# Shuijing725/CrowdNav_Prediction_AttnGraph

Measured on NVIDIA H100. Metric: env_steps_per_s_ppo_rollout, higher is better.
Workload: dtype f32

## Files before the change

### crowdnav_prediction_attngraph_b200/csrc/cn_gemm_tc.cu

```cuda
#include "cn_gemm_tc.h"

__global__ void cn_split_f16_kernel(const float* __restrict__ src, float scale, __half* __restrict__ hi,
                                    __half* __restrict__ lo, size_t count) {
  const size_t i = (size_t)blockIdx.x * blockDim.x + threadIdx.x;
  if (i >= count) return;
  const float x = fminf(fmaxf(src[i] * scale, -65504.0f), 65504.0f);
  const __half h = __float2half_rn(x);
  hi[i] = h;
  lo[i] = __float2half_rn(x - __half2float(h));
}

namespace {

typedef CUresult (*EncodeFn)(CUtensorMap*, CUtensorMapDataType, cuuint32_t, void*, const cuuint64_t*, const cuuint64_t*,
                             const cuuint32_t*, const cuuint32_t*, CUtensorMapInterleave, CUtensorMapSwizzle,
                             CUtensorMapL2promotion, CUtensorMapFloatOOBfill);

EncodeFn get_encode() {
  static EncodeFn fn = nullptr;
  if (!fn) {
    void* sym = nullptr;
    cudaDriverEntryPointQueryResult qres;
    if (cudaGetDriverEntryPoint("cuTensorMapEncodeTiled", &sym, cudaEnableDefault, &qres) == cudaSuccess &&
        qres == cudaDriverEntryPointSuccess)
      fn = reinterpret_cast<EncodeFn>(sym);
  }
  return fn;
}

int halloc16(CnLaunchCtx* c, __half** ptr, size_t count) {
  float* q = nullptr;
  int rc = palloc(c, &q, (count + 1) / 2);
// ... 78 lines not shown
  if (!rc) rc = tc_store_maps(v, rows, K);
  return rc;
}

void split16(CnLaunchCtx* c, cudaStream_t st, const float* src, float scale, __half* hi, __half* lo, size_t count) {
  cn_split_f16_kernel<<<(unsigned)((count + 255) / 256), 256, 0, st>>>(src, scale, hi, lo, count);
  c->launches += 1;
}

int tc_set_attrs() {
  cudaError_t e = cudaSuccess;
  for (int act = CN_ACT_NONE; act <= CN_ACT_TANH; ++act)
    for (int out = TC_OUT_F32; out <= TC_OUT_BOTH; ++out) {
      if (e == cudaSuccess)
        e = cudaFuncSetAttribute(tc_kernel<256>(act, out), cudaFuncAttributeMaxDynamicSharedMemorySize, TcCfg<256>::kSmemBytes);
      if (e == cudaSuccess)
        e = cudaFuncSetAttribute(tc_kernel<64>(act, out), cudaFuncAttributeMaxDynamicSharedMemorySize, TcCfg<64>::kSmemBytes);
    }
  if (e == cudaSuccess)
    e = cudaFuncSetAttribute(cn_gemm_tc_kernel<64, true>, cudaFuncAttributeMaxDynamicSharedMemorySize, TcCfg<64>::kSmemBytes);
  if (e == cudaSuccess)
    e = cudaFuncSetAttribute(cn_gemm_tc_kernel<256, false, CN_ACT_NONE, TC_OUT_GRU>,
                             cudaFuncAttributeMaxDynamicSharedMemorySize, TcCfg<256>::kSmemBytes);
  if (e != cudaSuccess) return cn_set_error("cudaFuncSetAttribute(tc): %s", cudaGetErrorString(e));
  return 0;
}

void gemm_tc(CnLaunchCtx* c, cudaStream_t st, const TcMat& A, const TcMat& B, int M, int N, int K, int bn, const float* bias,
             int act, const TcOut& o, const int* m_ptr, int act_lo, int act_hi, const int* m0_ptr) {
  TcEpilogue ep;
  memset(&ep, 0, sizeof(ep));
  ep.bias = bias; ep.inv_scale = 1.0f / 64.0f; ep.act = act; ep.act_lo = act_lo; ep.act_hi = act_hi;
  ep.c32 = o.c32; ep.ldc = o.ldc; ep.out_hi = o.oh; ep.out_lo = o.ol; ep.ldh = o.ldh; ep.m_ptr = m_ptr; ep.m0_ptr = m0_ptr;
  {
    static const int nostore = (getenv("CN_DBG_NOSTORE") && getenv("CN_DBG_NOSTORE")[0] == '1') ? 1 : 0;
    ep.dbg_nostore = nostore;
  }
  if (A.box_k != tc_box_k(bn) || B.box_k != tc_box_k(bn)) {
    if (!c->launch_error) {
      c->launch_error = true;
      cn_set_error("gemm_tc in stage '%s': operand boxes %d / %d wide, the BN = %d instance loads %d",
                   c->cur_stage ? c->cur_stage : "?", A.box_k, B.box_k, bn, tc_box_k(bn));
    }
    return;
  }
  const int out_kind = (o.c32 ? TC_OUT_F32 : 0) | (o.oh ? TC_OUT_F16 : 0);
// ... 35 lines not shown

void gemm_tc_gru(CnLaunchCtx* c, cudaStream_t st, const TcMat& A, const TcMat& B, int M, const float* bias,
                 const float* h_in, const float* mask, float* h_out, int group, int pitch, int off, __half* oh, __half* ol,
                 int ldh) {
  const int N = 4 * 256, K = 64 + 256;
  if (A.box_k != tc_box_k(256) || B.box_k != tc_box_k(256) || !bias || !h_out || !mask || group <= 0) {
    if (!c->launch_error) {
      c->launch_error = true;
      cn_set_error("gemm_tc_gru in stage '%s': operand boxes %d / %d wide (need %d), or a missing bias / mask / output",
                   c->cur_stage ? c->cur_stage : "?", A.box_k, B.box_k, tc_box_k(256));
    }
    return;
  }
  TcEpilogue ep;
  memset(&ep, 0, sizeof(ep));
  ep.bias = bias; ep.inv_scale = 1.0f / 64.0f; ep.act_hi = 1 << 30;
  ep.c32 = h_out; ep.ldc = 256; ep.out_hi = oh; ep.out_lo = ol; ep.ldh = ldh;
  ep.gru_h = h_in; ep.gru_mask = mask; ep.gru_group = group; ep.gru_pitch = pitch; ep.gru_off = off;
  static const CUtensorMap no_map = {};
  const int tiles = (N / 256) * ((M + TC_BM - 1) / TC_BM);
  dim3 grid(tiles < c->num_sms ? tiles : c->num_sms);
  launch_k(c, cn_gemm_tc_kernel<256, false, CN_ACT_NONE, TC_OUT_GRU>, grid, dim3(TC_THREADS), TcCfg<256>::kSmemBytes, st,
           A.mh, A.ml, B.mh, B.ml, M, N, K, ep, no_map, no_map, no_map);
}

int gemm_tc_promote(int num_sms, cudaStream_t st, const __half* ahi, const __half* alo, int a_rows, int a_pitch,
                    const __half* bhi, const __half* blo, int b_rows, int b_pitch, int Kd, float* C, int ldc,
                    const float* bias, int act, const float* inv_a, const float* inv_b, int ksplit) {
  const int bn = 64;
  if (b_rows % bn) return cn_set_error("cn_update gemm: output columns %d not a multiple of 64", b_rows);
  const int Kp = (Kd + TC_BK - 1) / TC_BK * TC_BK;
  CUtensorMap mah, mal, mbh, mbl;
  int rc = make_map(&mah, ahi, a_rows, Kd, TC_BM, a_pitch);
  if (!rc) rc = make_map(&mal, alo, a_rows, Kd, TC_BM, a_pitch);
  if (!rc) rc = make_map(&mbh, bhi, b_rows, Kd, bn, b_pitch);
  if (!rc) rc = make_map(&mbl, blo, b_rows, Kd, bn, b_pitch);
  if (rc) return rc;
  TcEpilogue ep;
  memset(&ep, 0, sizeof(ep));
  ep.bias = bias; ep.inv_scale = 1.0f; ep.act = act; ep.act_lo = 0; ep.act_hi = 1 << 30;
  ep.c32 = C; ep.ldc = ldc; ep.inv_scale_a = inv_a; ep.inv_scale_b = inv_b; ep.ksplit = ksplit;
  const int tiles = (b_rows / bn) * ((a_rows + TC_BM - 1) / TC_BM) * (ksplit > 1 ? ksplit : 1);
  const int grid = tiles < num_sms ? tiles : num_sms;
  static const CUtensorMap no_map = {};
  cn_gemm_tc_kernel<64, true><<<grid, TC_THREADS, TcCfg<64>::kSmemBytes, st>>>(mah, mal, mbh, mbl, a_rows, b_rows, Kp, ep,
                                                                                no_map, no_map, no_map);
// ... 29 lines not shown
  TcStoreMap sc, sh, sl;
  if (bn == 256) {
    if (!rc && dC) rc = make_store_map(&sc, dC, 4, M, N, N);
    if (!rc && out_hi) rc = make_store_map(&sh, out_hi, 2, M, N, ldh);
    if (!rc && out_hi) rc = make_store_map(&sl, out_lo, 2, M, N, ldh);
    o.sc = &sc; o.sh = &sh; o.sl = &sl;
  }
  if (!rc) {
    split16(&ctx, 0, dA, 1.0f, Af.hi, Af.lo, (size_t)M * a_pitch);
    split16(&ctx, 0, dW, 64.0f, B.hi, B.lo, (size_t)N * K);
    gemm_tc(&ctx, 0, A, B, M, N, K, bn, dbias, act, o, m_ptr, act_lo, act_hi > 0 ? act_hi : 1 << 30, m0_ptr);
    cudaError_t err = cudaDeviceSynchronize();
    if (err != cudaSuccess) rc = cn_set_error("cn_internal_gemm_tc_ex: %s", cudaGetErrorString(err));
    else if (ctx.launch_error) rc = 1;
  }
  cn_launch_free(&ctx);
  return rc;
}
int cn_internal_gemm_tc(const float* dA, const float* dW, const float* dbias, float* dC, int M, int N, int K, int act,
                        int bn) {
  return cn_internal_gemm_tc_ex(dA, dW, dbias, dC, M, N, K, act, bn, nullptr, nullptr, 0, 0, nullptr, nullptr, 0, 0, 0);
}

#ifdef CN_GEMM_TRACE
int cn_internal_gemm_trace(unsigned long long* dtrace, int cap) {
  g_tc_trace = dtrace; g_tc_trace_cap = dtrace ? cap : 0;
  return 0;
}
#endif

}
```

### crowdnav_prediction_attngraph_b200/csrc/cn_gemm_tc.cuh

```cuda
#pragma once
#include <cuda.h>
#include <cuda_fp16.h>
#include <cuda_runtime.h>
#include <stdint.h>

#include "cn_launch.cuh"

#define TC_BM 128
#define TC_BK 64
#define TC_CONSUMER_WARPS 8
#define TC_THREADS (128 + 32 * TC_CONSUMER_WARPS)

template <int BN>
struct TcCfg {
  static constexpr int kBK = (BN >= 256) ? 32 : TC_BK;
  static constexpr int kSwizzle = 2 * kBK;
  static constexpr int kStages = 4;
  static constexpr int kATile = TC_BM * kBK * 2;
  static constexpr int kBTile = BN * kBK * 2;
  static constexpr int kStageBytes = 2 * kATile + 2 * kBTile;
  static constexpr int kStoreBoxes = (BN >= 256) ? 2 : 0;
  static constexpr int kBoxBytes = 64 * 128;
  static constexpr int kStagingBytes = 2 * kStoreBoxes * kBoxBytes;
  static constexpr int kSmemBytes = kStages * kStageBytes + kStagingBytes + 256  + 1024 ;
// ... 384 lines not shown
#pragma unroll
      for (int k = 0; k < 2; ++k) {
        const int a = 4 * g + 2 * h + k;
        const float r = tc_sigmoid(fmaf(acc[a], inv_scale, __ldg(ep.bias + n0 + c + k)));
        const float z = tc_sigmoid(fmaf(acc[a + 32], inv_scale, __ldg(ep.bias + n0 + 64 + c + k)));
        const float gin = fmaf(acc[a + 64], inv_scale, __ldg(ep.bias + n0 + 128 + c + k));
        const float ghn = fmaf(acc[a + 96], inv_scale, __ldg(ep.bias + n0 + 192 + c + k));
        const float n = tanhf(gin + r * ghn);
        o[k] = (1.0f - z) * n + z * hv[k];
      }
      if (ep.dbg_nostore) continue;
      *reinterpret_cast<float2*>(ep.c32 + orow * 256 + u) = make_float2(o[0], o[1]);
      if (ep.out_hi) {
        uint32_t lo;
        const uint32_t hi = tc::split_pair_hi(o[0], o[1], &lo);
        const size_t q = (size_t)row * ep.ldh + u;
        *reinterpret_cast<uint32_t*>(ep.out_hi + q) = hi;
        *reinterpret_cast<uint32_t*>(ep.out_lo + q) = lo;
      }
    }
  }
}

template <int BN, bool PROMOTE = false, int ACT = 0, int OUT = TC_OUT_F32>
__global__ void __launch_bounds__(TC_THREADS, 1)
cn_gemm_tc_kernel(const __grid_constant__ CUtensorMap map_ahi, const __grid_constant__ CUtensorMap map_alo,
                  const __grid_constant__ CUtensorMap map_bhi, const __grid_constant__ CUtensorMap map_blo,
                  int M, int N, int K, TcEpilogue ep, const __grid_constant__ CUtensorMap map_c,
                  const __grid_constant__ CUtensorMap map_oh, const __grid_constant__ CUtensorMap map_ol) {
  cn_pdl_trigger();
  constexpr int TC_STAGES = TcCfg<BN>::kStages;
  constexpr int BK = TcCfg<BN>::kBK;
  constexpr int SW = TcCfg<BN>::kSwizzle;
  constexpr int TC_A_TILE_BYTES = TcCfg<BN>::kATile;
  constexpr int TC_B_TILE_BYTES = TcCfg<BN>::kBTile;
  constexpr int TC_STAGE_BYTES = TcCfg<BN>::kStageBytes;
  constexpr bool kTmaStore = !PROMOTE && BN == 256 && OUT != TC_OUT_GRU;
  static_assert(OUT != TC_OUT_GRU || (BN == 256 && !PROMOTE), "the GRU epilogue reads four 64-column gate blocks");
  static_assert(!PROMOTE || BK == 64, "PROMOTE sums 64-wide k-blocks");
  static_assert(!kTmaStore || TcCfg<BN>::kStoreBoxes > 0, "BN = 256 stages its output");
  extern __shared__ uint8_t tc_smem_raw[];
  const uint32_t raw = tc::smem_u32(tc_smem_raw);
  const uint32_t base = (raw + 1023u) & ~1023u;
  const uint32_t staging = base + TC_STAGES * TC_STAGE_BYTES;
  const uint32_t bar_base = staging + TcCfg<BN>::kStagingBytes;
  const uint32_t bar_full = bar_base, bar_empty = bar_base + 64;

  const int warp = threadIdx.x >> 5, lane = threadIdx.x & 31, wg = warp >> 2;
  const int num_kb = K / BK;

  if (threadIdx.x == 0) {
    for (int s = 0; s < TC_STAGES; ++s) {
      tc::mbar_init(bar_full + 8 * s, 1);
      tc::mbar_init(bar_empty + 8 * s, TC_CONSUMER_WARPS);
    }
    asm volatile("fence.mbarrier_init.release.cluster;" ::: "memory");
// ... 57 lines not shown
  sg.box = 0; sg.leader = (threadIdx.x & 127) == 0; sg.bar_id = wg;
  TC_TRACE(sg.waits = 0; sg.wait_clk = 0;)
  TC_TRACE(const bool tr = ep.trace && warp == 4 && lane == 0; int tr_n = 0;)
  for (int tile = blockIdx.x; tile < n_tiles; tile += gridDim.x) {
    const int mn = tile % n_mn, ks = tile / n_mn;
    const int m0 = m_lo + (mn / n_ntiles) * TC_BM, n0 = (mn % n_ntiles) * BN;
    const int kb0 = ks * kb_per, kb1 = (kb0 + kb_per < num_kb) ? kb0 + kb_per : num_kb;
    TC_TRACE(const uint64_t t_tile = tc::globaltimer(); uint64_t t_first = 0; uint32_t polls = 0;)
    float acc[BN / 2];
    float sum[PROMOTE ? BN / 2 : 1];
    if constexpr (PROMOTE) {
#pragma unroll
      for (int i = 0; i < BN / 2; ++i) sum[i] = 0.0f;
    }
    uint32_t prev = 0;
    for (int kb = kb0; kb < kb1; ++kb, ++it) {
      const uint32_t s = it % TC_STAGES, ph = (it / TC_STAGES) & 1u;
#ifdef CN_GEMM_TRACE
      polls += tc::mbar_wait_polls(bar_full + 8 * s, ph);
      if (kb == kb0) t_first = tc::globaltimer();
#else
      tc::mbar_wait(bar_full + 8 * s, ph);
#endif
      const uint32_t st = base + s * TC_STAGE_BYTES;
      const uint32_t a_hi = st + half * (TC_A_TILE_BYTES / 2), a_lo = a_hi + TC_A_TILE_BYTES,
                     b_hi = st + 2 * TC_A_TILE_BYTES, b_lo = b_hi + TC_B_TILE_BYTES;
      tc::fence_regs(acc);
      tc::wgmma_fence();
#pragma unroll
      for (int k = 0; k < BK / 16; ++k) {
        const uint32_t koff = k * 32;
        const uint64_t dah = tc::make_desc<SW>(a_hi + koff), dal = tc::make_desc<SW>(a_lo + koff);
        const uint64_t dbh = tc::make_desc<SW>(b_hi + koff), dbl = tc::make_desc<SW>(b_lo + koff);
        const bool first = k == 0 && (PROMOTE || kb == kb0);
        tc::wgmma_f16<BN>(acc, dah, dbh, first ? 0u : 1u);
        tc::wgmma_f16<BN>(acc, dah, dbl, 1u);
        tc::wgmma_f16<BN>(acc, dal, dbh, 1u);
      }
      tc::wgmma_commit();
      tc::fence_regs(acc);
      if constexpr (PROMOTE) {
        tc::wgmma_wait<0>();
        tc::fence_regs(acc);
        __syncwarp();
        if (lane == 0) tc::mbar_arrive(bar_empty + 8 * s);
#pragma unroll
        for (int i = 0; i < BN / 2; ++i) sum[i] += acc[i];
      } else {
        tc::wgmma_wait<1>();
        if (kb != kb0) {
          __syncwarp();
          if (lane == 0) tc::mbar_arrive(bar_empty + 8 * prev);
        }
        prev = s;
      }
    }
    if constexpr (PROMOTE) {
#pragma unroll
      for (int i = 0; i < BN / 2; ++i) acc[i] = sum[i];
    } else {
      tc::wgmma_wait<0>();
      tc::fence_regs(acc);
      __syncwarp();
// ... 44 lines not shown
        if (ep.c32) {
          float* c = ep.c32 + (size_t)row * ep.ldc + col;
          if (ksplit > 1) {
            atomicAdd(c, v0);
            atomicAdd(c + 1, v1);
          } else {
            *reinterpret_cast<float2*>(c) = make_float2(v0, v1);
          }
        }
        if (ep.out_hi) {
          uint32_t lo;
          const uint32_t hi = tc::split_pair_hi(v0, v1, &lo);
          const size_t o = (size_t)row * ep.ldh + col;
          *reinterpret_cast<uint32_t*>(ep.out_hi + o) = hi;
          *reinterpret_cast<uint32_t*>(ep.out_lo + o) = lo;
        }
      }
    }
  }
  if constexpr (kTmaStore) {
    if (sg.leader) tc::bulk_wait_all();
  }
}
```

### crowdnav_prediction_attngraph_b200/csrc/cn_gemm_tc.h

```cpp
#pragma once
#include <cuda.h>
#include <cuda_fp16.h>
#include <cuda_runtime.h>
#include <stdint.h>

#include "cn_gemm_tc.cuh"
#include "cn_launch.cuh"

struct TcStoreMap {
  CUtensorMap map;
  int rows = 0, cols = 0;
};

struct TcMat {
  __half *hi = nullptr, *lo = nullptr;
  CUtensorMap mh, ml;
  int pitch = 0;
  int box_k = 0;
  TcStoreMap sh, sl;
};

struct TcOut {
  float* c32 = nullptr; int ldc = 0;
  __half *oh = nullptr, *ol = nullptr; int ldh = 0;
// ... 2 lines not shown
inline TcOut out32(float* c, int ldc, const TcStoreMap* sc = nullptr) { TcOut o; o.c32 = c; o.ldc = ldc; o.sc = sc; return o; }
inline TcOut out16(const TcMat& t) { TcOut o; o.oh = t.hi; o.ol = t.lo; o.ldh = t.pitch; o.sh = &t.sh; o.sl = &t.sl; return o; }
inline TcOut out_both(float* c, int ldc, const TcMat& t) { TcOut o = out16(t); o.c32 = c; o.ldc = ldc; return o; }

inline int tc_box_k(int bn) { return bn == 256 ? TcCfg<256>::kBK : TcCfg<64>::kBK; }

inline bool tma_store_ok(const void* ptr, size_t pitch_bytes) { return ((uintptr_t)ptr % 16) == 0 && pitch_bytes % 16 == 0; }

int make_map(CUtensorMap* map, const __half* ptr, int rows, int K, int box_rows, int pitch, int box_k = TC_BK);
int make_store_map(TcStoreMap* s, const void* ptr, int esize, int rows, int cols, int pitch);
int tc_alloc(CnLaunchCtx* c, TcMat& t, int rows, int K, int box_rows, int box_k);
int tc_view(TcMat& v, const TcMat& src, int col0, int rows, int K, int box_rows);
void split16(CnLaunchCtx* c, cudaStream_t st, const float* src, float scale, __half* hi, __half* lo, size_t count);
int tc_set_attrs();

void gemm_tc(CnLaunchCtx* c, cudaStream_t st, const TcMat& A, const TcMat& B, int M, int N, int K, int bn, const float* bias,
             int act, const TcOut& o, const int* m_ptr = nullptr, int act_lo = 0, int act_hi = 1 << 30,
             const int* m0_ptr = nullptr);

void gemm_tc_gru(CnLaunchCtx* c, cudaStream_t st, const TcMat& A, const TcMat& B, int M, const float* bias,
                 const float* h_in, const float* mask, float* h_out, int group, int pitch, int off, __half* oh, __half* ol,
                 int ldh);

int gemm_tc_promote(int num_sms, cudaStream_t st, const __half* ahi, const __half* alo, int a_rows, int a_pitch,
                    const __half* bhi, const __half* blo, int b_rows, int b_pitch, int Kd, float* C, int ldc,
                    const float* bias, int act, const float* inv_a, const float* inv_b, int ksplit);
```

### crowdnav_prediction_attngraph_b200/csrc/cn_policy.cu

```cuda
#include <cuda_runtime.h>
#include <stdio.h>
#include <stdlib.h>
#include <string.h>
#include <map>
#include <string>
#include <vector>

#include "../../include/crowdnav_b200.h"
#include "cn_host_util.h"
#include "cn_gemm_tc.h"
#include "cn_launch.cuh"
#include "cn_policy_kernels.cuh"
#include "cn_qkv_attn.cuh"

struct cn_policy {
  cn_policy_config cfg;
  int N, H, Win, M;
  CnLaunchCtx lc;
  bool fuse_qkv;
  TcMat tWqkvH;
  CUtensorMap qa_ah, qa_al, qa_bh, qa_bl;
  float* bqkvH = nullptr;
  int* tile_tab = nullptr;
  cudaEvent_t ev_tiles;
  void (*attn_kernel)(const float*, const int*, const int*, const int*, const int*, float*, __half*, __half*);
  int attn_warps;
  int qkv_chunks;
  bool finalized;
  std::map<std::string, std::vector<float>> host;
  size_t ws_allocs;
  float *W1, *b1, *W2, *b2, *Wqkv, *bqkv, *Wos, *bos;
  float *Wr, *br, *Wet, *bet, *WsT, *bs, *Wa, *ba, *Wih, *bih, *Whh, *bhh, *Wo, *bo;
  float *Woac, *boac;
  float *Wac1, *bac1, *Wa2, *ba2, *Wc2, *bc2, *wv_, *bv, *Wm, *bm, *logstd;
  TcMat tW2, tWqkv, tWos, tWet, tWsT, tWa, tWih, tWhh, tWo, tWac1, tWoac, tWa2, tWc2;
  TcMat tE1, tE2, tAo;
  TcMat tRs, tT1, tTe, tWv, tH0, tH1, tOut, tAc1, tA1, tC1;
  cudaStream_t st2, st3;
  cudaEvent_t ev_fork, ev_join, ev_fork2, ev_join2, ev_fork3, ev_join3;
  bool profile;
  std::vector<cudaEvent_t> ev;
  int *row_start, *row_env, *mc;
  float *x16, *e1, *e2, *qkv, *ao, *sout, *xr, *rs, *t1, *u, *wv, *h0, *gi, *gh, *outb, *ac1, *a2, *c2;
  TcStoreMap qkv_st, sout_st;
};

void cn_hr_attention_dense(CnLaunchCtx* c, cudaStream_t st, const float* s_out, const float* u, const float* te, int ldte,
                           int te_off, const float* b_s, int env_pitch, int env_off, int N, int H, float* wv,
                           __half* wv_hi, __half* wv_lo, int ldwh) {
  launch_k(c, cn_hr_attention_kernel<true>, dim3((N + 3) / 4), dim3(128), 0, st, s_out, u, te, ldte, te_off, b_s,
// ... 69 lines not shown
    return cn_set_error("cn_policy_create: unsupported dims N=%d H=%d input=%d", cfg->num_envs, cfg->human_num,
                        cfg->input_size);
  int ndev = 0;
  cudaError_t err = cudaGetDeviceCount(&ndev);
  if (err != cudaSuccess || ndev == 0)
    return cn_set_error("cn_policy_create: no CUDA device (%s); this engine has no CPU fallback",
                        err == cudaSuccess ? "device count 0" : cudaGetErrorString(err));
  if (cfg->device < 0 || cfg->device >= ndev) return cn_set_error("cn_policy_create: bad device %d", cfg->device);
  cudaSetDevice(cfg->device);
  cn_policy* p = new cn_policy();
  p->cfg = *cfg;
  p->N = cfg->num_envs; p->H = cfg->human_num; p->Win = cfg->input_size; p->M = p->N * p->H;
  p->finalized = false; p->profile = false;
  cn_launch_init(&p->lc, cfg->device);
  {
    const char* qc = getenv("CN_QKV_CHUNKS");
    p->qkv_chunks = (qc && qc[0] == '2') ? 2 : 1;
    const char* ar = getenv("CN_ATTN_R");
    const int attn_r = ar ? atoi(ar) : 1;
    p->attn_kernel = attn_r == 1 ? cn_hh_attention_kernel<1, 4, 4> : (attn_r == 4 ? cn_hh_attention_kernel<4, 2, 2> : cn_hh_attention_kernel<2, 4, 4>);
    p->attn_warps = attn_r == 4 ? 2 : 4;
    const char* fq = getenv("CN_FUSE_QKV");
    p->fuse_qkv = cfg->gemm_mode == 1 && p->qkv_chunks == 1 && (fq && fq[0] == '1') && p->N <= QA_MAX_ENVS && p->H <= 128;
  }
  cudaEventCreateWithFlags(&p->ev_tiles, cudaEventDisableTiming);
  cudaStreamCreateWithFlags(&p->st2, cudaStreamNonBlocking);
  cudaStreamCreateWithFlags(&p->st3, cudaStreamNonBlocking);
  cudaEventCreateWithFlags(&p->ev_fork3, cudaEventDisableTiming);
  cudaEventCreateWithFlags(&p->ev_join3, cudaEventDisableTiming);
  cudaEventCreateWithFlags(&p->ev_fork, cudaEventDisableTiming);
  cudaEventCreateWithFlags(&p->ev_join, cudaEventDisableTiming);
  cudaEventCreateWithFlags(&p->ev_fork2, cudaEventDisableTiming);
  cudaEventCreateWithFlags(&p->ev_join2, cudaEventDisableTiming);
  const size_t M = (size_t)p->M, N = (size_t)p->N;
  const int Mi = p->M, Ni = p->N;
  int rc = 0;
#define WS(name, count) if (!rc) rc = palloc(&p->lc, &p->name, (count))
  {
    float* q = nullptr;
    if (!rc) rc = palloc(&p->lc, &q, N + 2);
    p->row_start = reinterpret_cast<int*>(q);
    if (!rc) rc = palloc(&p->lc, &q, 4);
    p->mc = reinterpret_cast<int*>(q);
    if (!rc) rc = palloc(&p->lc, &q, M + 1);
    p->row_env = reinterpret_cast<int*>(q);
    if (!rc) rc = palloc(&p->lc, &q, 2 * N + 4);
    p->tile_tab = reinterpret_cast<int*>(q);
  }
  WS(x16, M * 16); WS(e1, M * 128); WS(e2, M * 512); WS(qkv, M * 1536); WS(ao, M * 512); WS(sout, M * 256);
  WS(xr, N * 16); WS(rs, N * 256); WS(t1, N * 128); WS(u, N * 256); WS(wv, N * 256); WS(h0, N * 128);
  WS(gi, N * 384); WS(gh, N * 384); WS(outb, N * 256); WS(ac1, N * 512); WS(a2, N * 256); WS(c2, N * 256);
#undef WS
  if (!rc && cfg->gemm_mode == 1) {
    rc = tc_alloc(&p->lc, p->tE1, Mi, 128, TC_BM, tc_box_k(256));
    if (!rc) rc = tc_alloc(&p->lc, p->tE2, Mi, 512, TC_BM, tc_box_k(256));
    if (!rc) rc = tc_alloc(&p->lc, p->tAo, Mi, 512, TC_BM, tc_box_k(256));
    if (!rc) rc = tc_alloc(&p->lc, p->tRs, Ni, 256, TC_BM, tc_box_k(64));
    if (!rc) rc = tc_alloc(&p->lc, p->tT1, Ni, 128, TC_BM, tc_box_k(64));
    if (!rc) rc = tc_view(p->tTe, p->tT1, 64, Ni, 64, TC_BM);
    if (!rc) rc = tc_alloc(&p->lc, p->tWv, Ni, 256, TC_BM, tc_box_k(64));
    if (!rc) rc = tc_alloc(&p->lc, p->tH0, Ni, 128, TC_BM, tc_box_k(64));
    if (!rc) rc = tc_alloc(&p->lc, p->tH1, Ni, 128, TC_BM, tc_box_k(64));
    if (!rc) rc = tc_alloc(&p->lc, p->tOut, Ni, 256, TC_BM, tc_box_k(64));
    if (!rc) rc = tc_alloc(&p->lc, p->tAc1, Ni, 512, TC_BM, tc_box_k(64));
    if (!rc) rc = tc_view(p->tA1, p->tAc1, 0, Ni, 256, TC_BM);
    if (!rc) rc = tc_view(p->tC1, p->tAc1, 256, Ni, 256, TC_BM);
    if (!rc) rc = make_store_map(&p->qkv_st, p->qkv, 4, Mi, 1536, 1536);
    if (!rc) rc = make_store_map(&p->sout_st, p->sout, 4, Mi, 256, 256);
    if (!rc) rc = tc_set_attrs();
    if (!rc) {
// ... 160 lines not shown
      split16(&p->lc, st, wh, 64.0f, p->tWqkvH.hi, p->tWqkvH.lo, (size_t)1536 * 512);
    }
  }
  cudaError_t err = cudaStreamSynchronize(st);
  if (err != cudaSuccess) return cn_set_error("cn_policy_finalize: %s", cudaGetErrorString(err));
  p->finalized = true;
  return 0;
}

int cn_policy_act(cn_policy* p, const cn_act_ptrs* d, void* stream) {
  if (!p || !d) return cn_set_error("cn_policy_act: null argument");
  if (!p->finalized) return cn_set_error("cn_policy_act: call cn_policy_finalize after setting parameters");
  if (!d->robot_node || !d->temporal_edges || !d->spatial_edges || !d->detected_human_num || !d->h_in || !d->masks ||
      !d->value || !d->action || !d->log_prob || !d->h_out)
    return cn_set_error("cn_policy_act: missing input/output pointer");
  CnDeviceGuard guard(p->cfg.device);
  cudaStream_t st = (cudaStream_t)stream;
  const int N = p->N, H = p->H, M = p->M;
  const bool tcm = p->cfg.gemm_mode == 1;
  const int* mc = p->mc;
  const int ALL = 1 << 30;
  mark(p, st, 0);
  {
    launch_k(&p->lc, cn_row_offsets_kernel, dim3(1), dim3(1024), 0, st, d->detected_human_num, N, H, p->row_start, p->mc);
    const int total = (!tcm && M * 16 > N * 128) ? M * 16 : N * 128;
    launch_k(&p->lc, cn_pack_inputs_kernel, dim3((total + 255) / 256), dim3(256), 0, st, d->spatial_edges, p->Win, H, N, p->row_start, p->row_env,
                                                               tcm ? nullptr : p->x16,
                                                               d->temporal_edges, d->robot_node, d->h_in, d->masks, p->xr,
                                                               p->h0, tcm ? p->tH0.hi : nullptr, tcm ? p->tH0.lo : nullptr);
  }
  cudaStream_t s2 = p->st2;
  cudaEventRecord(p->ev_fork, st);
  cudaStreamWaitEvent(s2, p->ev_fork, 0);
  if (p->fuse_qkv) {
    cn_qkv_tiles_kernel<<<1, 1024, 0, s2>>>(p->row_start, N, p->tile_tab);
    p->lc.launches += 1;
    cudaEventRecord(p->ev_tiles, s2);
  }
  if (tcm) {
    gemm(p, s2, p->xr, 16, p->Wr, 16, p->br, nullptr, 256, N, 256, 16, CN_ACT_RELU, 0, ALL, nullptr, p->tRs.hi, p->tRs.lo);
    gemm_tc(&p->lc, s2, p->tRs, p->tWet, N, 128, 256, 64, p->bet, CN_ACT_RELU, out_both(p->t1, 128, p->tT1), nullptr, 0, 64);
    gemm_tc(&p->lc, s2, p->tTe, p->tWsT, N, 256, 64, 64, nullptr, CN_ACT_NONE, out32(p->u, 256));
    gemm_tc(&p->lc, s2, p->tH0, p->tWhh, N, 384, 128, 64, p->bhh, CN_ACT_NONE, out32(p->gh, 384));
  } else {
    gemm(p, s2, p->xr, 16, p->Wr, 16, p->br, p->rs, 256, N, 256, 16, CN_ACT_RELU);
    gemm(p, s2, p->rs, 256, p->Wet, 256, p->bet, p->t1, 128, N, 128, 256, CN_ACT_RELU, 0, 64);
    gemm(p, s2, p->t1 + 64, 128, p->WsT, 64, nullptr, p->u, 256, N, 256, 64, CN_ACT_NONE);
    gemm(p, s2, p->h0, 128, p->Whh, 128, p->bhh, p->gh, 384, N, 384, 128, CN_ACT_NONE);
  }
  cudaEventRecord(p->ev_join, s2);
  mark(p, st, 1);
  if (tcm) {
    launch_k(&p->lc, cn_embed1_kernel, dim3(p->lc.num_sms * 6), dim3(256), 0, st, d->spatial_edges, p->Win, H, p->row_start, p->row_env, p->mc, p->W1, p->b1,
                                                     p->tE1.hi, p->tE1.lo);
  } else gemm(p, st, p->x16, 16, p->W1, 16, p->b1, p->e1, 128, M, 128, 16, CN_ACT_RELU, 0, ALL, mc);
  mark(p, st, 2);
  if (tcm) gemm_tc(&p->lc, st, p->tE1, p->tW2, M, 512, 128, 256, p->b2, CN_ACT_RELU, out16(p->tE2), mc);
  else gemm(p, st, p->e1, 128, p->W2, 128, p->b2, p->e2, 512, M, 512, 128, CN_ACT_RELU, 0, ALL, mc);
  mark(p, st, 3);
  if (tcm) {
    const int* mid = p->row_start + N / 2;
    __half* ah = p->tAo.hi;
    __half* al = p->tAo.lo;
    if (p->fuse_qkv) {
      cudaStreamWaitEvent(st, p->ev_tiles, 0);
      launch_k(&p->lc, cn_qkv_attn_kernel, dim3(p->lc.num_sms), dim3(QA_THREADS), QA_SMEM_BYTES, st, p->qa_ah, p->qa_al, p->qa_bh,
               p->qa_bl, p->bqkvH, 1.0f / 64.0f, p->tile_tab, p->row_start, p->row_env, ah, al,
               getenv("CN_QA_DBG") ? atoi(getenv("CN_QA_DBG")) : 0);
      mark(p, st, 4);
    } else if (p->qkv_chunks == 1) {
      gemm_tc(&p->lc, st, p->tE2, p->tWqkv, M, 1536, 512, 256, p->bqkv, CN_ACT_NONE, out32(p->qkv, 1536, &p->qkv_st), mc);
      mark(p, st, 4);
      launch_k(&p->lc, p->attn_kernel, dim3(p->lc.num_sms * 64 / p->attn_warps), dim3(p->attn_warps * 32), 0, st, p->qkv, p->row_start, p->row_env, mc, nullptr,
                                                                             nullptr, ah, al);
    } else {
    gemm_tc(&p->lc, st, p->tE2, p->tWqkv, M, 1536, 512, 256, p->bqkv, CN_ACT_NONE, out32(p->qkv, 1536, &p->qkv_st), mid);
    cudaEventRecord(p->ev_fork3, st);
    cudaStreamWaitEvent(p->st3, p->ev_fork3, 0);
    launch_k(&p->lc, p->attn_kernel, dim3(p->lc.num_sms * 32 / p->attn_warps), dim3(p->attn_warps * 32), 0, p->st3, p->qkv, p->row_start, p->row_env, mid, nullptr,
                                                                              nullptr, ah, al);
    cudaEventRecord(p->ev_join3, p->st3);
    gemm_tc(&p->lc, st, p->tE2, p->tWqkv, M, 1536, 512, 256, p->bqkv, CN_ACT_NONE, out32(p->qkv, 1536, &p->qkv_st), mc, 0, 1 << 30, mid);
    mark(p, st, 4);
    launch_k(&p->lc, p->attn_kernel, dim3(p->lc.num_sms * 64 / p->attn_warps), dim3(p->attn_warps * 32), 0, st, p->qkv, p->row_start, p->row_env, mc, mid, nullptr,
                                                                           ah, al);
    cudaStreamWaitEvent(st, p->ev_join3, 0);
    }
  } else {
    gemm(p, st, p->e2, 512, p->Wqkv, 512, p->bqkv, p->qkv, 1536, M, 1536, 512, CN_ACT_NONE, 0, ALL, mc);
    mark(p, st, 4);
    launch_k(&p->lc, p->attn_kernel, dim3(p->lc.num_sms * 64 / p->attn_warps), dim3(p->attn_warps * 32), 0, st, p->qkv, p->row_start, p->row_env, p->mc, nullptr,
                                                                           p->ao, nullptr, nullptr);
  }
  mark(p, st, 5);
// ... 109 lines not shown
```

### crowdnav_prediction_attngraph_b200/csrc/cn_policy_kernels.cuh

```cuda
#pragma once
#include <cuda_fp16.h>
#include <cuda_runtime.h>
#include <stdint.h>

#include "cn_launch.cuh"

#define CN_GEMM_BM 128
#define CN_GEMM_BN 128
#define CN_GEMM_BK 16
#define CN_GEMM_PAD 4

__device__ __forceinline__ float cn_apply_act(float v, int act) {
  if (act == CN_ACT_RELU) return v > 0.0f ? v : 0.0f;
  if (act == CN_ACT_TANH) return tanhf(v);
  return v;
}

__global__ void __launch_bounds__(256) cn_gemm_f32_kernel(const float* __restrict__ A, int lda,
                                                          const float* __restrict__ W, int ldw,
                                                          const float* __restrict__ bias, float* __restrict__ Cout,
                                                          int ldc, int M, int N, int K, int act, int act_lo,
                                                          int act_hi, const int* __restrict__ m_ptr,
                                                          __half* __restrict__ out_hi, __half* __restrict__ out_lo) {
  cn_pdl_prologue();
// ... 108 lines not shown
      }
    }
  }
}

__global__ void cn_fold_mm_kernel(const float* __restrict__ A, const float* __restrict__ B, float* __restrict__ Cm,
                                  int M, int N, int K) {
  const int n = blockIdx.x * blockDim.x + threadIdx.x, m = blockIdx.y;
  if (n >= N || m >= M) return;
  double acc = 0.0;
  for (int k = 0; k < K; ++k) acc += (double)A[(size_t)m * K + k] * (double)B[(size_t)k * N + n];
  Cm[(size_t)m * N + n] = (float)acc;
}
__global__ void cn_fold_mv_kernel(const float* __restrict__ A, const float* __restrict__ b, const float* __restrict__ d,
                                  float* __restrict__ c, int M, int K) {
  const int m = blockIdx.x * blockDim.x + threadIdx.x;
  if (m >= M) return;
  double acc = d ? (double)d[m] : 0.0;
  for (int k = 0; k < K; ++k) acc += (double)A[(size_t)m * K + k] * (double)b[k];
  c[m] = (float)acc;
}

__global__ void __launch_bounds__(1024) cn_row_offsets_kernel(const float* __restrict__ detected, int N, int H,
                                                              int* __restrict__ row_start, int* __restrict__ mc) {
  cn_pdl_prologue();
  __shared__ int warp_sums[32];
  __shared__ int carry;
  const int tid = threadIdx.x, lane = tid & 31, warp = tid >> 5;
  if (tid == 0) carry = 0;
  __syncthreads();
  for (int base = 0; base < N; base += 1024) {
    const int e = base + tid;
    int n = 0;
    if (e < N) { n = (int)detected[e]; n = n < 1 ? 1 : (n > H ? H : n); }
    int x = n;
#pragma unroll
    for (int o = 1; o < 32; o <<= 1) { const int y = __shfl_up_sync(0xffffffffu, x, o); if (lane >= o) x += y; }
    if (lane == 31) warp_sums[warp] = x;
    __syncthreads();
    if (warp == 0) {
      int w = warp_sums[lane];
#pragma unroll
      for (int o = 1; o < 32; o <<= 1) { const int y = __shfl_up_sync(0xffffffffu, w, o); if (lane >= o) w += y; }
      warp_sums[lane] = w;
    }
    __syncthreads();
    const int incl = x + (warp > 0 ? warp_sums[warp - 1] : 0) + carry;
    if (e < N) row_start[e] = incl - n;
    __syncthreads();
    if (tid == 1023) carry = incl;
    __syncthreads();
// ... 378 lines not shown
```

Baseline: 6.851 million.

## Fuse E2 and QKV tensor-core GEMMs into one persistent chained kernel

Adds a persistent warp-specialized kernel that runs the E1→E2 (ReLU, f16 split output) GEMM and the E2→QKV GEMM in one launch. Work items come from an atomic counter with a lagged schedule, and per-row-block release/acquire flags let QKV tiles start as soon as their E2 rows are written, instead of waiting for a full kernel boundary. The counters are zeroed inside the row-offsets kernel, and the new path is on by default when the gemm mode allows it. This saves a launch and the tail between the two GEMMs, at the cost of inter-CTA spin waits and dependence on forward progress across CTAs.

```diff
diff --git a/crowdnav_prediction_attngraph_b200/csrc/cn_gemm_tc.cu b/crowdnav_prediction_attngraph_b200/csrc/cn_gemm_tc.cu
--- a/crowdnav_prediction_attngraph_b200/csrc/cn_gemm_tc.cu
+++ b/crowdnav_prediction_attngraph_b200/csrc/cn_gemm_tc.cu
@@ -8,6 +8,103 @@
   const __half h = __float2half_rn(x);
   hi[i] = h;
   lo[i] = __float2half_rn(x - __half2float(h));
+}
+
+__global__ void __launch_bounds__(TC_THREADS, 1)
+cn_human_chain_kernel(const __grid_constant__ TcChainMaps maps, const TcChainArgs a) {
+  cn_pdl_trigger();
+  constexpr int BN = 256, STAGES = TcCfg<BN>::kStages, BK = TcCfg<BN>::kBK;
+  constexpr int A_TILE = TcCfg<BN>::kATile, B_TILE = TcCfg<BN>::kBTile, STAGE_BYTES = TcCfg<BN>::kStageBytes;
+  extern __shared__ uint8_t tc_smem_raw[];
+  const uint32_t raw = tc::smem_u32(tc_smem_raw);
+  const uint32_t base = (raw + 1023u) & ~1023u;
+  const uint32_t staging = base + STAGES * STAGE_BYTES;
+  const uint32_t bar_base = staging + TcCfg<BN>::kStagingBytes;
+  const uint32_t bar_full = bar_base, bar_empty = bar_base + 64, tags = bar_base + 128;
+  const int warp = threadIdx.x >> 5, lane = threadIdx.x & 31, wg = warp >> 2;
+
+  if (threadIdx.x == 0) {
+    for (int s = 0; s < STAGES; ++s) {
+      tc::mbar_init(bar_full + 8 * s, 1);
+      tc::mbar_init(bar_empty + 8 * s, TC_CONSUMER_WARPS);
+    }
+    asm volatile("fence.mbarrier_init.release.cluster;" ::: "memory");
+    const CUtensorMap* m = &maps.e1h;
+    for (int i = 0; i < (int)(sizeof(TcChainMaps) / sizeof(CUtensorMap)); ++i)
+      asm volatile("prefetch.tensormap [%0];" ::"l"(m + i) : "memory");
+  }
+  __syncthreads();
+  cn_pdl_wait();
+  const int nb = (cn_ld_after_wait(a.mc) + TC_BM - 1) / TC_BM;
+
+  if (wg == 0) {
+    tc::setmaxnreg_dec<40>();
+    if (threadIdx.x == 0) {
+      uint32_t it = 0;
+      while (true) {
+        const TcChainItem w = tc_chain_item((int)atomicAdd(a.work, 1u), nb);
+        if (w.kind == TC_CHAIN_SKIP) continue;
+        const uint32_t tag = (uint32_t)w.kind | ((uint32_t)w.col << 2) | ((uint32_t)w.blk << 5);
+        if (w.kind == TC_CHAIN_END) {
+          const uint32_t s = it % STAGES, ph = (it / STAGES) & 1u;
+          tc::mbar_wait(bar_empty + 8 * s, ph ^ 1u);
+          tc::st_shared_b32(tags + 4 * s, tag);
+          tc::mbar_arrive(bar_full + 8 * s);
+          break;
+        }
+        const CUtensorMap *ah = &maps.e1h, *al = &maps.e1l, *bh = &maps.w2h, *bl = &maps.w2l;
+        int nkb = 128 / BK;
+        if (w.kind == TC_CHAIN_Q) {
+          tc::acquire_wait(a.work + 1 + w.blk, TC_CHAIN_DONE_E);
+          tc::fence_proxy_async_global();
+          ah = &maps.e2h; al = &maps.e2l; bh = &maps.wqh; bl = &maps.wql; nkb = 512 / BK;
+        }
+        const int m0 = w.blk * TC_BM, n0 = w.col * BN;
+        for (int kb = 0; kb < nkb; ++kb, ++it) {
+          const uint32_t s = it % STAGES, ph = (it / STAGES) & 1u;
+          tc::mbar_wait(bar_empty + 8 * s, ph ^ 1u);
+          if (kb == 0) tc::st_shared_b32(tags + 4 * s, tag);
+          const uint32_t full = bar_full + 8 * s;
+          tc::mbar_expect_tx(full, STAGE_BYTES);
+          const uint32_t st = base + s * STAGE_BYTES;
+          tc::tma_load_2d(st, ah, full, kb * BK, m0);
+          tc::tma_load_2d(st + A_TILE, al, full, kb * BK, m0);
+          tc::tma_load_2d(st + 2 * A_TILE, bh, full, kb * BK, n0);
+          tc::tma_load_2d(st + 2 * A_TILE + B_TILE, bl, full, kb * BK, n0);
+        }
+      }
+    }
+    return;
+  }
+  tc::setmaxnreg_inc<232>();
+  const int half = wg - 1;
+  const int wr = 16 * (warp & 3) + (lane >> 2);
+  TcStaging sg;
+  sg.base = staging + half * TcCfg<BN>::kStoreBoxes * TcCfg<BN>::kBoxBytes;
+  sg.box = 0; sg.leader = (threadIdx.x & 127) == 0; sg.bar_id = wg;
+  TC_TRACE(sg.waits = 0; sg.wait_clk = 0;)
+  uint32_t it = 0;
+  while (true) {
+    const uint32_t s = it % STAGES, ph = (it / STAGES) & 1u;
+    tc::mbar_wait(bar_full + 8 * s, ph);
+    const uint32_t tag = tc::ld_shared_b32(tags + 4 * s);
+    const int kind = (int)(tag & 3u), col = (int)((tag >> 2) & 7u), blk = (int)(tag >> 5);
+    if (kind == TC_CHAIN_END) break;
+    const int m0 = blk * TC_BM, n0 = col * BN;
+    if (kind == TC_CHAIN_E) {
+      tc_chain_gemm<CN_ACT_RELU, TC_OUT_F16>(it, 128 / BK, m0, n0, a.ep_e, base, bar_full, bar_empty, half, wr, lane, sg,
+                                             nullptr, &maps.e2sh, &maps.e2sl);
+      if (sg.leader) {
+        tc::bulk_wait_all();
+        tc::fence_proxy_async_global();
+        tc::release_add(a.work + 1 + blk);
+      }
+    } else {
+      tc_chain_gemm<CN_ACT_NONE, TC_OUT_F32>(it, 512 / BK, m0, n0, a.ep_q, base, bar_full, bar_empty, half, wr, lane, sg,
+                                             &maps.qkv_s, nullptr, nullptr);
+    }
+  }
+  if (sg.leader) tc::bulk_wait_all();
 }
 
 namespace {
@@ -132,6 +229,8 @@
   if (e == cudaSuccess)
     e = cudaFuncSetAttribute(cn_gemm_tc_kernel<256, false, CN_ACT_NONE, TC_OUT_GRU>,
                              cudaFuncAttributeMaxDynamicSharedMemorySize, TcCfg<256>::kSmemBytes);
+  if (e == cudaSuccess)
+    e = cudaFuncSetAttribute(cn_human_chain_kernel, cudaFuncAttributeMaxDynamicSharedMemorySize, TcCfg<256>::kSmemBytes);
   if (e != cudaSuccess) return cn_set_error("cudaFuncSetAttribute(tc): %s", cudaGetErrorString(e));
   return 0;
 }
@@ -213,6 +312,35 @@
   dim3 grid(tiles < c->num_sms ? tiles : c->num_sms);
   launch_k(c, cn_gemm_tc_kernel<256, false, CN_ACT_NONE, TC_OUT_GRU>, grid, dim3(TC_THREADS), TcCfg<256>::kSmemBytes, st,
            A.mh, A.ml, B.mh, B.ml, M, N, K, ep, no_map, no_map, no_map);
+}
+
+void gemm_tc_human_chain(CnLaunchCtx* c, cudaStream_t st, const TcMat& e1, const TcMat& w2, const float* b2, const TcMat& e2,
+                         const TcMat& wqkv, const float* bqkv, const TcStoreMap& qkv_st, const int* mc, unsigned* work,
+                         int M) {
+  const int box = tc_box_k(256);
+  if (e1.box_k != box || w2.box_k != box || e2.box_k != box || wqkv.box_k != box || e2.sh.rows != M ||
+      e2.sh.cols != 512 || e2.sl.rows != M || e2.sl.cols != 512 || qkv_st.rows != M || qkv_st.cols != 1536) {
+    if (!c->launch_error) {
+      c->launch_error = true;
+      cn_set_error("human chain in stage '%s': operand boxes must be %d wide and the outputs need TMA store maps of "
+                   "[%d x 512 / 1536]", c->cur_stage ? c->cur_stage : "?", box, M);
+    }
+    return;
+  }
+  TcChainMaps maps;
+  maps.e1h = e1.mh; maps.e1l = e1.ml; maps.w2h = w2.mh; maps.w2l = w2.ml;
+  maps.e2h = e2.mh; maps.e2l = e2.ml; maps.wqh = wqkv.mh; maps.wql = wqkv.ml;
+  maps.e2sh = e2.sh.map; maps.e2sl = e2.sl.map; maps.qkv_s = qkv_st.map;
+  TcChainArgs a;
+  memset(&a, 0, sizeof(a));
+  a.mc = mc; a.work = work;
+  TcEpilogue* eps[2] = {&a.ep_e, &a.ep_q};
+  const float* bias[2] = {b2, bqkv};
+  const int act[2] = {CN_ACT_RELU, CN_ACT_NONE};
+  for (int i = 0; i < 2; ++i) {
+    eps[i]->bias = bias[i]; eps[i]->inv_scale = 1.0f / 64.0f; eps[i]->act = act[i]; eps[i]->act_lo = 0; eps[i]->act_hi = 1 << 30;
+  }
+  launch_k(c, cn_human_chain_kernel, dim3(c->num_sms), dim3(TC_THREADS), TcCfg<256>::kSmemBytes, st, maps, a);
 }
 
 int gemm_tc_promote(int num_sms, cudaStream_t st, const __half* ahi, const __half* alo, int a_rows, int a_pitch,
@@ -288,6 +416,22 @@
   return cn_internal_gemm_tc_ex(dA, dW, dbias, dC, M, N, K, act, bn, nullptr, nullptr, 0, 0, nullptr, nullptr, 0, 0, 0);
 }
 
+int cn_internal_chain_schedule(int mc, int* out, int cap) {
+  if (!out || mc < 0) return -1;
+  const int nb = (mc + TC_BM - 1) / TC_BM;
+  int n = 0;
+  for (int idx = 0;; ++idx) {
+    const TcChainItem w = tc_chain_item(idx, nb);
+    if (w.kind == TC_CHAIN_END) break;
+    if (w.kind == TC_CHAIN_SKIP) continue;
+    if (n < cap) {
+      out[3 * n] = w.kind; out[3 * n + 1] = w.blk; out[3 * n + 2] = w.col;
+    }
+    ++n;
+  }
+  return n;
+}
+
 #ifdef CN_GEMM_TRACE
 int cn_internal_gemm_trace(unsigned long long* dtrace, int cap) {
   g_tc_trace = dtrace; g_tc_trace_cap = dtrace ? cap : 0;
diff --git a/crowdnav_prediction_attngraph_b200/csrc/cn_gemm_tc.cuh b/crowdnav_prediction_attngraph_b200/csrc/cn_gemm_tc.cuh
--- a/crowdnav_prediction_attngraph_b200/csrc/cn_gemm_tc.cuh
+++ b/crowdnav_prediction_attngraph_b200/csrc/cn_gemm_tc.cuh
@@ -430,6 +430,27 @@
   }
 }
 
+template <int BN>
+__device__ __forceinline__ void tc_kblock_mma(float (&acc)[BN / 2], uint32_t st, int half, bool first) {
+  constexpr int BK = TcCfg<BN>::kBK, SW = TcCfg<BN>::kSwizzle;
+  constexpr int TC_A_TILE_BYTES = TcCfg<BN>::kATile, TC_B_TILE_BYTES = TcCfg<BN>::kBTile;
+  const uint32_t a_hi = st + half * (TC_A_TILE_BYTES / 2), a_lo = a_hi + TC_A_TILE_BYTES,
+                 b_hi = st + 2 * TC_A_TILE_BYTES, b_lo = b_hi + TC_B_TILE_BYTES;
+  tc::fence_regs(acc);
+  tc::wgmma_fence();
+#pragma unroll
+  for (int k = 0; k < BK / 16; ++k) {
+    const uint32_t koff = k * 32;
+    const uint64_t dah = tc::make_desc<SW>(a_hi + koff), dal = tc::make_desc<SW>(a_lo + koff);
+    const uint64_t dbh = tc::make_desc<SW>(b_hi + koff), dbl = tc::make_desc<SW>(b_lo + koff);
+    tc::wgmma_f16<BN>(acc, dah, dbh, (first && k == 0) ? 0u : 1u);
+    tc::wgmma_f16<BN>(acc, dah, dbl, 1u);
+    tc::wgmma_f16<BN>(acc, dal, dbh, 1u);
+  }
+  tc::wgmma_commit();
+  tc::fence_regs(acc);
+}
+
 template <int BN, bool PROMOTE = false, int ACT = 0, int OUT = TC_OUT_F32>
 __global__ void __launch_bounds__(TC_THREADS, 1)
 cn_gemm_tc_kernel(const __grid_constant__ CUtensorMap map_ahi, const __grid_constant__ CUtensorMap map_alo,
@@ -439,7 +460,6 @@
   cn_pdl_trigger();
   constexpr int TC_STAGES = TcCfg<BN>::kStages;
   constexpr int BK = TcCfg<BN>::kBK;
-  constexpr int SW = TcCfg<BN>::kSwizzle;
   constexpr int TC_A_TILE_BYTES = TcCfg<BN>::kATile;
   constexpr int TC_B_TILE_BYTES = TcCfg<BN>::kBTile;
   constexpr int TC_STAGE_BYTES = TcCfg<BN>::kStageBytes;
@@ -543,23 +563,7 @@
 #else
       tc::mbar_wait(bar_full + 8 * s, ph);
 #endif
-      const uint32_t st = base + s * TC_STAGE_BYTES;
-      const uint32_t a_hi = st + half * (TC_A_TILE_BYTES / 2), a_lo = a_hi + TC_A_TILE_BYTES,
-                     b_hi = st + 2 * TC_A_TILE_BYTES, b_lo = b_hi + TC_B_TILE_BYTES;
-      tc::fence_regs(acc);
-      tc::wgmma_fence();
-#pragma unroll
-      for (int k = 0; k < BK / 16; ++k) {
-        const uint32_t koff = k * 32;
-        const uint64_t dah = tc::make_desc<SW>(a_hi + koff), dal = tc::make_desc<SW>(a_lo + koff);
-        const uint64_t dbh = tc::make_desc<SW>(b_hi + koff), dbl = tc::make_desc<SW>(b_lo + koff);
-        const bool first = k == 0 && (PROMOTE || kb == kb0);
-        tc::wgmma_f16<BN>(acc, dah, dbh, first ? 0u : 1u);
-        tc::wgmma_f16<BN>(acc, dah, dbl, 1u);
-        tc::wgmma_f16<BN>(acc, dal, dbh, 1u);
-      }
-      tc::wgmma_commit();
-      tc::fence_regs(acc);
+      tc_kblock_mma<BN>(acc, base + s * TC_STAGE_BYTES, half, PROMOTE || kb == kb0);
       if constexpr (PROMOTE) {
         tc::wgmma_wait<0>();
         tc::fence_regs(acc);
@@ -650,3 +654,83 @@
     if (sg.leader) tc::bulk_wait_all();
   }
 }
+
+enum { TC_CHAIN_E = 0, TC_CHAIN_Q = 1, TC_CHAIN_SKIP = 2, TC_CHAIN_END = 3 };
+#define TC_CHAIN_SLOTS 8
+#define TC_CHAIN_DONE_E 4
+#define TC_CHAIN_LAG 32
+
+struct TcChainItem {
+  int kind, blk, col;
+};
+
+__host__ __device__ inline TcChainItem tc_chain_item(int idx, int nb) {
+  TcChainItem w;
+  const int rounds = nb > 0 ? nb + TC_CHAIN_LAG : 0;
+  if (idx >= rounds * TC_CHAIN_SLOTS) { w.kind = TC_CHAIN_END; w.blk = 0; w.col = 0; return w; }
+  const int t = idx / TC_CHAIN_SLOTS, s = idx % TC_CHAIN_SLOTS;
+  if (s < 2) { w.kind = TC_CHAIN_E; w.blk = t; w.col = s; }
+  else { w.kind = TC_CHAIN_Q; w.blk = t - TC_CHAIN_LAG; w.col = s - 2; }
+  if (w.blk < 0 || w.blk >= nb) w.kind = TC_CHAIN_SKIP;
+  return w;
+}
+
+struct TcChainMaps {
+  CUtensorMap e1h, e1l, w2h, w2l;
+  CUtensorMap e2h, e2l, wqh, wql;
+  CUtensorMap e2sh, e2sl, qkv_s;
+};
+struct TcChainArgs {
+  const int* mc;
+  unsigned* work;
+  TcEpilogue ep_e, ep_q;
+};
+
+namespace tc {
+__device__ __forceinline__ void fence_proxy_async_global() { asm volatile("fence.proxy.async.global;" ::: "memory"); }
+__device__ __forceinline__ void release_add(unsigned* p) {
+  asm volatile("red.release.gpu.global.add.u32 [%0], 1;" ::"l"(p) : "memory");
+}
+__device__ __forceinline__ void acquire_wait(const unsigned* p, unsigned target) {
+  unsigned v;
+  while (true) {
+    asm volatile("ld.acquire.gpu.global.u32 %0, [%1];" : "=r"(v) : "l"(p) : "memory");
+    if (v >= target) return;
+    __nanosleep(32);
+  }
+}
+__device__ __forceinline__ uint32_t ld_shared_b32(uint32_t addr) {
+  uint32_t v;
+  asm volatile("ld.shared.b32 %0, [%1];" : "=r"(v) : "r"(addr) : "memory");
+  return v;
+}
+}
+
+template <int ACT, int OUT>
+__device__ __forceinline__ void tc_chain_gemm(uint32_t& it, int nkb, int m0, int n0, const TcEpilogue& ep, uint32_t base,
+                                              uint32_t bar_full, uint32_t bar_empty, int half, int wr, int lane,
+                                              TcStaging& sg, const CUtensorMap* map_c, const CUtensorMap* map_oh,
+                                              const CUtensorMap* map_ol) {
+  constexpr int STAGES = TcCfg<256>::kStages, STAGE_BYTES = TcCfg<256>::kStageBytes;
+  float acc[128];
+  uint32_t prev = 0;
+  for (int kb = 0; kb < nkb; ++kb, ++it) {
+    const uint32_t s = it % STAGES, ph = (it / STAGES) & 1u;
+    if (kb > 0) tc::mbar_wait(bar_full + 8 * s, ph);
+    tc_kblock_mma<256>(acc, base + s * STAGE_BYTES, half, kb == 0);
+    tc::wgmma_wait<1>();
+    if (kb != 0) {
+      __syncwarp();
+      if (lane == 0) tc::mbar_arrive(bar_empty + 8 * prev);
+    }
+    prev = s;
+  }
+  tc::wgmma_wait<0>();
+  tc::fence_regs(acc);
+  __syncwarp();
+  if (lane == 0) tc::mbar_arrive(bar_empty + 8 * prev);
+  tc_epilogue_tma<ACT, OUT>(acc, ep, ep.inv_scale, n0, m0 + 64 * half, wr, lane, sg, map_c, map_oh, map_ol);
+}
+
+__global__ void __launch_bounds__(TC_THREADS, 1)
+cn_human_chain_kernel(const __grid_constant__ TcChainMaps maps, const TcChainArgs a);
diff --git a/crowdnav_prediction_attngraph_b200/csrc/cn_gemm_tc.h b/crowdnav_prediction_attngraph_b200/csrc/cn_gemm_tc.h
--- a/crowdnav_prediction_attngraph_b200/csrc/cn_gemm_tc.h
+++ b/crowdnav_prediction_attngraph_b200/csrc/cn_gemm_tc.h
@@ -48,6 +48,11 @@
                  const float* h_in, const float* mask, float* h_out, int group, int pitch, int off, __half* oh, __half* ol,
                  int ldh);
 
+void gemm_tc_human_chain(CnLaunchCtx* c, cudaStream_t st, const TcMat& e1, const TcMat& w2, const float* b2, const TcMat& e2,
+                         const TcMat& wqkv, const float* bqkv, const TcStoreMap& qkv_st, const int* mc, unsigned* work,
+                         int M);
+inline int tc_chain_work_words(int M) { return 1 + (M + TC_BM - 1) / TC_BM; }
+
 int gemm_tc_promote(int num_sms, cudaStream_t st, const __half* ahi, const __half* alo, int a_rows, int a_pitch,
                     const __half* bhi, const __half* blo, int b_rows, int b_pitch, int Kd, float* C, int ldc,
                     const float* bias, int act, const float* inv_a, const float* inv_b, int ksplit);
diff --git a/crowdnav_prediction_attngraph_b200/csrc/cn_policy.cu b/crowdnav_prediction_attngraph_b200/csrc/cn_policy.cu
--- a/crowdnav_prediction_attngraph_b200/csrc/cn_policy.cu
+++ b/crowdnav_prediction_attngraph_b200/csrc/cn_policy.cu
@@ -26,6 +26,8 @@
   void (*attn_kernel)(const float*, const int*, const int*, const int*, const int*, float*, __half*, __half*);
   int attn_warps;
   int qkv_chunks;
+  bool human_chain;
+  unsigned* chain_work = nullptr;
   bool finalized;
   std::map<std::string, std::vector<float>> host;
   size_t ws_allocs;
@@ -141,6 +143,8 @@
     p->attn_warps = attn_r == 4 ? 2 : 4;
     const char* fq = getenv("CN_FUSE_QKV");
     p->fuse_qkv = cfg->gemm_mode == 1 && p->qkv_chunks == 1 && (fq && fq[0] == '1') && p->N <= QA_MAX_ENVS && p->H <= 128;
+    const char* hc = getenv("CN_HUMAN_CHAIN");
+    p->human_chain = cfg->gemm_mode == 1 && p->qkv_chunks == 1 && !p->fuse_qkv && !(hc && hc[0] == '0');
   }
   cudaEventCreateWithFlags(&p->ev_tiles, cudaEventDisableTiming);
   cudaStreamCreateWithFlags(&p->st2, cudaStreamNonBlocking);
@@ -165,6 +169,10 @@
     p->row_env = reinterpret_cast<int*>(q);
     if (!rc) rc = palloc(&p->lc, &q, 2 * N + 4);
     p->tile_tab = reinterpret_cast<int*>(q);
+    if (!rc && p->human_chain) {
+      rc = palloc(&p->lc, &q, tc_chain_work_words(p->M));
+      p->chain_work = reinterpret_cast<unsigned*>(q);
+    }
   }
   WS(x16, M * 16); WS(e1, M * 128); WS(e2, M * 512); WS(qkv, M * 1536); WS(ao, M * 512); WS(sout, M * 256);
   WS(xr, N * 16); WS(rs, N * 256); WS(t1, N * 128); WS(u, N * 256); WS(wv, N * 256); WS(h0, N * 128);
@@ -371,7 +379,8 @@
   const int ALL = 1 << 30;
   mark(p, st, 0);
   {
-    launch_k(&p->lc, cn_row_offsets_kernel, dim3(1), dim3(1024), 0, st, d->detected_human_num, N, H, p->row_start, p->mc);
+    launch_k(&p->lc, cn_row_offsets_kernel, dim3(1), dim3(1024), 0, st, d->detected_human_num, N, H, p->row_start, p->mc,
+             p->chain_work, p->human_chain ? tc_chain_work_words(M) : 0);
     const int total = (!tcm && M * 16 > N * 128) ? M * 16 : N * 128;
     launch_k(&p->lc, cn_pack_inputs_kernel, dim3((total + 255) / 256), dim3(256), 0, st, d->spatial_edges, p->Win, H, N, p->row_start, p->row_env,
                                                                tcm ? nullptr : p->x16,
@@ -404,9 +413,14 @@
                                                      p->tE1.hi, p->tE1.lo);
   } else gemm(p, st, p->x16, 16, p->W1, 16, p->b1, p->e1, 128, M, 128, 16, CN_ACT_RELU, 0, ALL, mc);
   mark(p, st, 2);
-  if (tcm) gemm_tc(&p->lc, st, p->tE1, p->tW2, M, 512, 128, 256, p->b2, CN_ACT_RELU, out16(p->tE2), mc);
-  else gemm(p, st, p->e1, 128, p->W2, 128, p->b2, p->e2, 512, M, 512, 128, CN_ACT_RELU, 0, ALL, mc);
-  mark(p, st, 3);
+  if (p->human_chain) {
+    mark(p, st, 3);
+    gemm_tc_human_chain(&p->lc, st, p->tE1, p->tW2, p->b2, p->tE2, p->tWqkv, p->bqkv, p->qkv_st, mc, p->chain_work, M);
+  } else {
+    if (tcm) gemm_tc(&p->lc, st, p->tE1, p->tW2, M, 512, 128, 256, p->b2, CN_ACT_RELU, out16(p->tE2), mc);
+    else gemm(p, st, p->e1, 128, p->W2, 128, p->b2, p->e2, 512, M, 512, 128, CN_ACT_RELU, 0, ALL, mc);
+    mark(p, st, 3);
+  }
   if (tcm) {
     const int* mid = p->row_start + N / 2;
     __half* ah = p->tAo.hi;
@@ -418,7 +432,8 @@
                getenv("CN_QA_DBG") ? atoi(getenv("CN_QA_DBG")) : 0);
       mark(p, st, 4);
     } else if (p->qkv_chunks == 1) {
-      gemm_tc(&p->lc, st, p->tE2, p->tWqkv, M, 1536, 512, 256, p->bqkv, CN_ACT_NONE, out32(p->qkv, 1536, &p->qkv_st), mc);
+      if (!p->human_chain)
+        gemm_tc(&p->lc, st, p->tE2, p->tWqkv, M, 1536, 512, 256, p->bqkv, CN_ACT_NONE, out32(p->qkv, 1536, &p->qkv_st), mc);
       mark(p, st, 4);
       launch_k(&p->lc, p->attn_kernel, dim3(p->lc.num_sms * 64 / p->attn_warps), dim3(p->attn_warps * 32), 0, st, p->qkv, p->row_start, p->row_env, mc, nullptr,
                                                                              nullptr, ah, al);
diff --git a/crowdnav_prediction_attngraph_b200/csrc/cn_policy_kernels.cuh b/crowdnav_prediction_attngraph_b200/csrc/cn_policy_kernels.cuh
--- a/crowdnav_prediction_attngraph_b200/csrc/cn_policy_kernels.cuh
+++ b/crowdnav_prediction_attngraph_b200/csrc/cn_policy_kernels.cuh
@@ -154,11 +154,14 @@
 }
 
 __global__ void __launch_bounds__(1024) cn_row_offsets_kernel(const float* __restrict__ detected, int N, int H,
-                                                              int* __restrict__ row_start, int* __restrict__ mc) {
+                                                              int* __restrict__ row_start, int* __restrict__ mc,
+                                                              unsigned* __restrict__ chain_work, int nwork) {
   cn_pdl_prologue();
   __shared__ int warp_sums[32];
   __shared__ int carry;
   const int tid = threadIdx.x, lane = tid & 31, warp = tid >> 5;
+  if (chain_work)
+    for (int i = tid; i < nwork; i += 1024) chain_work[i] = 0u;
   if (tid == 0) carry = 0;
   __syncthreads();
   for (int base = 0; base < N; base += 1024) {
```

Measured after the change: 6.856 million (median of 6 runs). About the same (+0.1%).
